# Blackgaurd/pathtracer-cpp

Hardware: AMD Instinct MI355X
Metric: Mray/s (all bounces) + achieved HBM GB/s, Cornell 1024² 10k spp depth-5 (higher is better)
Workload: dtype f32

## Files before the change

### include/pt_hip_debug.h

```cpp
#ifndef PT_HIP_DEBUG_H
#define PT_HIP_DEBUG_H

#include "pt_hip.h"

#ifdef __cplusplus
extern "C" {
#endif

int pt_debug_math(int device, int which, const float* in, int n, float* out);
int pt_debug_sweep(int device, int which, uint32_t lo_bits, uint32_t hi_bits, uint64_t* mismatches,
                   uint32_t* first_bad);
int pt_debug_rgb8(int device, const float* linear_rgb, int32_t res_x, int32_t res_y, float gamma, uint8_t* rgb8);
int pt_debug_rccl_failover(int32_t n_devices, int32_t fail_step, int64_t* out);
int pt_debug_wide_verify(const pt_scene* scene, int32_t width);
int pt_debug_pack_hash(const pt_scene* scene, uint64_t* hash);
int pt_rtc_check(const pt_scene* scene, char* src_out, size_t cap);
int pt_debug_rtc_start(const pt_scene* scene);
int64_t pt_debug_rtc_cache(int32_t op);

int pt_debug_ctx_flags(const pt_ctx* ctx, int32_t out[5]);
int pt_debug_ctx_plan(const pt_ctx* ctx, int64_t out[24]);
int pt_debug_walk_placement(int32_t num_nodes, int32_t num_tris, int32_t tree_depth, int32_t tri_f4,
                            int32_t rec_rows, uint64_t lds_usable, int32_t out[4]);
int pt_debug_scene_dark(const pt_scene* scene);
int pt_debug_emit_reject(const float* box6, const float* org, const float* dir, int64_t n, uint8_t* out);
int pt_debug_emit_slab_reject(const float* box6, const float* org, const float* inv, int64_t n, uint8_t* out);
int pt_debug_emit_box(const pt_scene* scene, float out[6]);
int pt_debug_ctx_emit_reject(const pt_ctx* ctx, int32_t* on, float box[6], uint64_t* early);
int pt_debug_ray_stack(int32_t which, int32_t count, int32_t n, int32_t reserve, int32_t flag);
int64_t pt_debug_counter(int32_t which);

#ifdef __cplusplus
}
#endif
#endif
```

### pathtracer-cpp_amd/csrc/pt_kernel.hip

```cpp
#include <hip/hip_runtime.h>

#include <stdint.h>
#include <stdio.h>
#include <stdlib.h>
#include <string.h>

#include <algorithm>
#include <chrono>
#include <future>
#include <map>
#include <memory>
#include <mutex>
#include <string>
#include <thread>
#include <vector>

#include <atomic>

#include "pt_grad.h"
#include "pt_hip_debug.h"
#include "pt_launch.h"
#include "pt_moments.h"
#include "pt_rtc.h"
#include "pt_trace.h"
// ... 297 lines not shown
    float4* d_nrm = nullptr;
    float4* d_umats = nullptr;
    int32_t* d_rank_tri = nullptr;
    std::vector<f4> flat_host;
    FlatLeaves flat_tab;
    int flat_boxes_padded = 0;
    PackedScene meta;
    bool have_scene = false;
    bool has_specular = false;
    bool albedo_x2 = false;
    bool dark = false;
    EmitBox emit;
    uint64_t last_early = 0;
    void* flat_fast = nullptr;
    int flat_boxes = 0;
    bool rtc_requested = false;
    float* d_radiance = nullptr;
    size_t radiance_floats = 0;
    uint32_t* d_flags = nullptr;
    size_t flags_words = 0;
    float* d_accum = nullptr;
    size_t accum_floats = 0;
    float* d_out = nullptr;
    size_t out_floats = 0;
    unsigned long long* d_ctr = nullptr;
    unsigned long long* d_stamps = nullptr;
    int* d_xstack = nullptr;
    size_t xstack_ints = 0;
    uint8_t* d_rgb8 = nullptr;
    size_t rgb8_bytes = 0;
// ... 228 lines not shown
int batch_at(const RenderPlan& P, int s0) {
    const int left = P.spp - s0;
    if (P.tail <= 0 || left <= P.tail) return std::min(P.batch, left);
    return left <= P.batch + P.tail ? left - P.tail : P.batch;
}

size_t flat_lds_bytes(const pt_ctx* c, const RenderPlan& P, int queue) {
    return sizeof(float4) * (size_t)(3 + 2) * c->meta.num_tris + sizeof(uint16_t) * (size_t)queue * (kBlock / kWave) +
           (sizeof(uint16_t) + sizeof(float)) * (size_t)kBlock * P.rec + sizeof(unsigned long long) * kBlock +
           (sizeof(float4) + sizeof(uint32_t)) * kBlock + P.box_tab_bytes;
}

void plan_flat(const pt_ctx* c, RenderPlan& P) {
    P.pairs = !hook_off("PT_PAIRS");
    P.box_tab_bytes = (sizeof(uint16_t) * (size_t)c->flat_boxes + 3) & ~(size_t)3;
    int queue = P.pairs ? 512 : 0;
    const char* pq = hook_env("PT_PAIR_QUEUE");
    if (P.pairs && pq && *pq) {
        queue = std::max(1, std::min(queue, atoi(pq)));
    } else if (P.pairs && c->lds_usable > 0) {
        auto blocks = [&](int q) { return std::min(8, lds_blocks(c->lds_usable, flat_lds_bytes(c, P, q))); };
        const int want = blocks(kPairQueueMin);
        while (queue > kPairQueueMin && blocks(queue) < want) queue -= 32;
    }
    P.pair_queue = (queue + 3) & ~3;
    P.lds_scene = true;
    P.lds_bytes = flat_lds_bytes(c, P, P.pair_queue);
}

size_t wide_lds_bytes(const pt_ctx* c, const RenderPlan& P, int top) {
// ... 310 lines not shown
            fprintf(stderr,
                    "[stamps] wide timeline: span %.3f ms, first exhaustion at %.3f ms, last wave end %.3f ms after it, "
                    "last exhaustion %.3f ms after it | mean wave life %.3f ms, mean end - own exhaustion %.3f ms\n",
                    (hs[18] - t0) * 1e-5, (ex0 - t0) * 1e-5, (hs[18] - ex0) * 1e-5, (hs[22] - ex0) * 1e-5,
                    hs[20] / w * 1e-5, hs[21] / w * 1e-5);
        }
        const double tot = (double)(hs[0] + hs[5] + hs[3] + hs[4]);
        if (!wide) fprintf(stderr,
                "[stamps] waves %llu  cycles/wave %.3g  start %.1f%%  intersect %.1f%% (box mask %.1f%%, "
                "pair phase %.1f%%)  shade %.1f%%  fold %.1f%%\n",
                hs[6], tot / (double)(hs[6] ? hs[6] : 1), 100 * hs[0] / tot, 100 * hs[5] / tot,
                100 * hs[1] / tot, 100 * hs[2] / tot, 100 * hs[3] / tot, 100 * hs[4] / tot);
        const double it = (double)(hs[7] ? hs[7] : 1);
        if (!wide)
            fprintf(stderr, "[stamps] per flat wave-iteration: pairs %.1f, pair rounds %.2f, max pairs of a lane %.2f, "
                    "rays credited %.2f (%llu wave-iterations)\n",
                hs[8] / it, hs[9] / it, hs[10] / it, (double)h_ctr[1] / it, hs[7]);
        if (!wide)
            fprintf(stderr, "[stamps] camera-ray generator: %.4f runs per wave-iteration, %.2f lanes per run (%llu runs)\n",
                    hs[11] / it, (double)hs[12] / (double)(hs[11] ? hs[11] : 1), hs[11]);
    }
}
#endif

int kernel_path_of(const pt_ctx* c, const RenderPlan& P) {
    return P.use_rtc                ? PT_PATH_FLAT_RTC
           : P.flat && c->flat_fast ? PT_PATH_FLAT_TABLE_FAST
           : P.flat                 ? PT_PATH_FLAT_TABLE
           : P.wide                 ? PT_PATH_WIDE
           : P.lds_scene            ? PT_PATH_TREE_LDS
                                    : PT_PATH_TREE_GLOBAL;
}
// ... 364 lines not shown
    ps.nrm.clear();
    ps.umats.clear();
    ps.nodes.clear();
    ps.tris.clear();
    ps.mats.clear();
    ps.rank_tri.clear();
    c->has_specular = specular;
    c->dark = dark;
    c->emit = emit;
    c->albedo_x2 = false;
    c->flat_fast = nullptr;
    if (flat_eligible(ps) && !hook_off("PT_FLAT_FAST") && leaves_single(ps.leaves, ps.num_leaves) && ps.coords_small &&
        c->dark && albedo_x2)
        c->flat_fast = flat_fast_kernel(specular, ps.num_leaves <= 32);
    c->flat_boxes = 0;
    c->rtc_requested = false;
    c->flat_host = ps.leaves;
    ps.leaves.clear();
    c->meta = ps;
    build_flat_table(c);
    c->rtc_flat = nullptr;
    c->rtc_job = RtcFuture();
    c->rtc_src.clear();
    c->rtc_status = "not a flat scene";
    if (want_rtc) {
        c->rtc_src = std::move(src);
        c->albedo_x2 = albedo_x2;
        c->rtc_requested = true;
        c->flat_boxes = flat_box_pairs(c->flat_host, ps.num_leaves);
        c->rtc_job = job;
        c->rtc_status = "compiling";
        const char* w = hook_env("PT_RTC_WAIT");
        if ((w && *w == '1') || !rtc_async_ready()) rtc_resolve(c, true);
    }
    c->have_scene = true;
    return PT_OK;
}

int pt_rtc_wait(void) { return rtc_wait_all(); }

int pt_ctx_prepare(pt_ctx* c) {
    if (!c) return set_error(PT_E_ARG, "context is NULL");
    if (int rc = ctx_ready(c)) return rc;
    if (c->rtc_job.valid()) {
// ... 1051 lines not shown
    return PT_OK;
}

int pt_debug_ray_stack(int32_t which, int32_t count, int32_t n, int32_t reserve, int32_t flag) {
    switch (which) {
        case 0: return ray_stack_generate(count, n, reserve, flag != 0) ? 1 : 0;
        case 1: return ray_stack_filled(count, n);
        case 2: return ray_stack_dry(count, n) ? 1 : 0;
        case 3: return ray_stack_slot(count, n);
        case 4: return ray_stack_taken(count, n);
        case 5: return ray_stack_done(flag != 0, count, n != 0) ? 1 : 0;
    }
    return set_error(PT_E_ARG, "pt_debug_ray_stack: which = %d", which);
}

int pt_debug_ctx_plan(const pt_ctx* c, int64_t out[24]) {
    if (!c || !out) return set_error(PT_E_ARG, "pt_debug_ctx_plan: NULL argument");
    memcpy(out, c->last_plan, sizeof(c->last_plan));
    return PT_OK;
}

int pt_debug_scene_dark(const pt_scene* scene) {
    PackedScene ps;
    const int rc = pack_scene(scene, ps);
    if (rc) return rc;
    return scene_dark(ps) ? 1 : 0;
}

int pt_debug_math(int device, int which, const float* in, int n, float* out) {
    if (!in || !out || n <= 0 || which < 0 || which > 2) return set_error(PT_E_ARG, "pt_debug_math: bad argument");
// ... 53 lines not shown
```

### pathtracer-cpp_amd/csrc/pt_rtc.h

```cpp
#pragma once

#include <hip/hip_runtime_api.h>

#include <future>
#include <memory>
#include <string>
#include <vector>

#include "pt_internal.h"

namespace pt {

struct RtcCode {
    std::vector<char> code;
    std::string status;
    std::string disk_key;
};
typedef std::shared_future<std::shared_ptr<const RtcCode>> RtcFuture;

int flat_box_pairs(const std::vector<f4>& leaves, int n, std::vector<uint16_t>* tab = nullptr);
bool leaves_single(const std::vector<f4>& leaves, int n);
std::string rtc_flat_source(const std::vector<f4>& leaves, int n, bool specular, bool tri_fast, bool albedo_x2,
                            bool dark, const EmitBox& emit);
RtcFuture rtc_job(const std::string& src);
bool rtc_async_ready();
int rtc_wait_all();
hipFunction_t rtc_load(int device, const std::string& src, const RtcCode& code, std::string& status);

}
```

### pathtracer-cpp_amd/csrc/pt_rtc.hip

```cpp
#include <hip/hip_runtime.h>
#include <hip/hiprtc.h>

#include <dlfcn.h>
#include <errno.h>
#include <fcntl.h>
#include <link.h>
#include <signal.h>
#include <spawn.h>
#include <stdint.h>
#include <stdio.h>
#include <stdlib.h>
#include <string.h>
#include <sys/socket.h>
#include <sys/stat.h>
#include <sys/wait.h>
#include <unistd.h>

#include <algorithm>
#include <atomic>
#include <chrono>
#include <fstream>
#include <future>
#include <limits>
#include <map>
// ... 4 lines not shown
#include <string>
#include <thread>
#include <vector>

extern char** environ;

#include "pt_hip_debug.h"
#include "pt_launch.h"
#include "pt_rtc.h"
#include "pt_sha256.h"
#include "pt_trace.h"

extern "C" const char* pt_rtc_src_trace;
extern "C" const char* pt_rtc_src_math;
extern "C" const char* pt_rtc_src_stack;
extern "C" const char* pt_rtc_src_hip;

namespace pt {

namespace {

std::string hexf(float v) {
    char b[64];
    snprintf(b, sizeof(b), "%af", (double)v);
    return b;
}

std::string litf(float v) {
    if (v == std::numeric_limits<float>::infinity()) return "__builtin_inff()";
    if (v == -std::numeric_limits<float>::infinity()) return "-__builtin_inff()";
    return hexf(v);
}

}

int flat_box_pairs(const std::vector<f4>& leaves, int n, std::vector<uint16_t>* tab) {
    const char* e = hook_env("PT_BOX_PAIRS");
    if (!e || *e != '1') return 0;
    std::map<std::vector<uint32_t>, int> box_id;
    std::vector<std::vector<int>> box_leaves;
    for (int k = 0; k < n; k++) {
        const f4 a = leaves[2 * k], b = leaves[2 * k + 1];
        if (__builtin_bit_cast(int, b.z) != k || __builtin_bit_cast(int, b.w) != k) return 0;
        const std::vector<uint32_t> key = {f2u(a.x), f2u(a.y), f2u(a.z), f2u(a.w), f2u(b.x), f2u(b.y)};
        auto it = box_id.find(key);
        if (it == box_id.end()) {
            it = box_id.emplace(key, (int)box_leaves.size()).first;
            box_leaves.emplace_back();
        }
        box_leaves[it->second].push_back(k);
    }
    for (const auto& l : box_leaves)
        if (l.size() > 2 || l.back() > 254) return 0;
    if (tab) {
        tab->clear();
        for (const auto& l : box_leaves) tab->push_back((uint16_t)(l[0] | ((l.size() > 1 ? l[1] : 0xff) << 8)));
    }
    return (int)box_leaves.size();
}

bool leaves_single(const std::vector<f4>& leaves, int n) {
    for (int k = 0; k < n; k++)
        if (__builtin_bit_cast(int, leaves[2 * k + 1].z) != k || __builtin_bit_cast(int, leaves[2 * k + 1].w) != k)
            return false;
    return true;
}

namespace {

std::string flat_mask_source(const std::vector<f4>& leaves, int n, bool specular, bool tri_fast, bool albedo_x2,
                             bool dark, const EmitBox& emit) {
    std::vector<std::map<uint32_t, int>> planes(3);
    auto plane = [&](int ax, float c) {
// ... 112 lines not shown
            acc += bit;
    }
    acc += "#if PT_MULTI_LEAF_OR\n";
    for (size_t i = 0; i < box_bits.size(); i++) {
        const unsigned long long m = box_bits[i];
        if (__builtin_popcountll(m) < 2) continue;
        const std::string bal = "__builtin_amdgcn_ballot_w64(b" + std::to_string(i) + ")";
        if ((uint32_t)m)
            acc += "        lo = or_if_bit(lo, " + std::to_string((uint32_t)m) + "u, " + bal + ");\n";
        if ((uint32_t)(m >> 32))
            acc += "        hi = or_if_bit(hi, " + std::to_string((uint32_t)(m >> 32)) + "u, " + bal + ");\n";
    }
    acc += "#endif\n";
    acc += "#endif\n";
    std::vector<uint16_t> box_tab;
    const int nbox = flat_box_pairs(leaves, n, &box_tab);
    if (nbox > 0) {
        std::string chain = "        lo = 0;\n        hi = 0;\n";
        for (int u = nbox - 1; u >= 0; u--) {
            const char* w = u >= 32 ? "hi" : "lo";
            chain += std::string("        ") + w + " = shl1_add_bit(" + w + ", __builtin_amdgcn_ballot_w64(b" +
                     std::to_string(u) + "));\n";
        }
        acc = "#if KBOX\n        uint32_t lo, hi;\n" + chain + "#else\n" + acc + "#endif\n";
    }
    acc += "        const unsigned long long m = ((unsigned long long)hi << 32) | lo;\n";
    const bool single = leaves_single(leaves, n);
    const bool sign = tri_fast;
    std::string tabs = "{";
    for (size_t u = 0; u < box_tab.size(); u++) tabs += (u ? ", " : "") + std::to_string(box_tab[u]) + "u";
    tabs += box_tab.empty() ? "0u}" : "}";
    std::string rej = "    using EmitRej = NoEmitReject;\n";
    if (emit.on)
        rej = "    struct EmitRej {\n        static constexpr bool kCompiled = true;\n"
              "        __device__ __forceinline__ static bool on() { return true; }\n"
              "        __device__ __forceinline__ static bool rejected(v3 o, v3 d) {\n"
              "            return emit_reject(v3{" + litf(emit.lo[0]) + ", " + litf(emit.lo[1]) + ", " + litf(emit.lo[2]) +
              "}, v3{" + litf(emit.hi[0]) + ", " + litf(emit.hi[1]) + ", " + litf(emit.hi[2]) + "}, o, d);\n"
              "        }\n"
              "        static constexpr bool kSlab = !PT_EMIT_SIGN_ONLY;\n"
              "        __device__ __forceinline__ static bool rejected_slab(v3 o, v3, v3 inv) {\n"
              "            return emit_slab_reject(v3{" + litf(emit.lo[0]) + ", " + litf(emit.lo[1]) + ", " + litf(emit.lo[2]) +
              "}, v3{" + litf(emit.hi[0]) + ", " + litf(emit.hi[1]) + ", " + litf(emit.hi[2]) + "}, o, inv);\n"
              "        }\n    };\n";
    return std::string("#ifndef PT_FLAT_SIGN_MASK\n#define PT_FLAT_SIGN_MASK 0\n#endif\n#define KSIGN (PT_FLAT_SIGN_MASK && ") +
           (sign ? "1" : "0") + ")\n" + "#define KBOX " + (nbox > 0 ? "(!KSIGN)" : "0") + "\n" +
           "namespace pt {\nstruct SceneBoxMask {\n    static constexpr bool kSignMask = KSIGN;\n"
           "    static constexpr bool kBoxPairs = KBOX;\n    static constexpr bool kCamInvGen = PT_CAM_INV == 2;\n"
           "    static constexpr bool kRayStack = PT_RAY_STACK != 0;\n"
           "    static constexpr int kBoxes = " + std::to_string(nbox) +
           ";\n    static constexpr uint16_t kBoxTab[" + std::to_string(std::max<size_t>(1, box_tab.size())) + "] = " + tabs +
           ";\n    static constexpr bool kMask32 = " +
           (n <= 32 ? "true" : "false") + ";\n    static constexpr bool kSingleTri = " + (single ? "true" : "false") +
           ";\n    static constexpr bool kSpecular = " + (specular ? "true" : "false") +
           ";\n    static constexpr bool kTriFast = " + (tri_fast ? "true" : "false") +
           ";\n    static constexpr bool kAlbedoX2 = " + (albedo_x2 ? "true" : "false") +
           ";\n    static constexpr bool kDarkKnown = true;\n    static constexpr bool kDark = " + (dark ? "true" : "false") +
           ";\n" + rej + "    __device__ __forceinline__ static unsigned long long "
           "mask(const TraceArgs&, v3 o, v3 inv) {\n" +
           body + tests + acc + "        return m;\n    }\n};\n}  // namespace pt\n";
}

struct RtcCache {
    std::mutex mu;
    std::map<std::string, RtcFuture> code;
    std::map<std::pair<int, std::string>, hipFunction_t> funcs;
    std::set<std::string> refused;
// ... 97 lines not shown
        dlclose(h);
    }
    const std::string rtc = lib_of(reinterpret_cast<const void*>(&hiprtcCompileProgram));
    if (!rtc.empty()) libs.push_back(rtc);
    if (runtime) {
        const std::string hip = lib_of(reinterpret_cast<const void*>(&hipModuleLoadData));
        if (!hip.empty()) libs.push_back(hip);
    }
    return libs;
}

std::string rtc_key(const std::string& src) {
    Sha256 k;
    k.update("pathtracer-amd hipRTC code object v1");
    k.update(src.c_str(), src.size() + 1);
    for (const char* h : {pt_rtc_src_trace, pt_rtc_src_math, pt_rtc_src_stack, pt_rtc_src_hip}) k.update(h, strlen(h) + 1);
    for (const std::string& f : rtc_flags()) k.update(f.c_str(), f.size() + 1);
    int maj = 0, mnr = 0;
    (void)hiprtcVersion(&maj, &mnr);
    k.update(std::to_string(maj) + "." + std::to_string(mnr));
    k.update(std::to_string(HIP_VERSION) + " " + HIP_VERSION_GITHASH);
    for (const std::string& lib : rtc_compiler_libs(true)) {
        struct stat st;
        const bool ok = stat(lib.c_str(), &st) == 0;
        k.update(lib + " " + (ok ? std::to_string((long long)st.st_size) + " " + std::to_string((long long)st.st_mtime) : "?"));
    }
    return k.hex();
}

bool rtc_dir_private(const std::string& dir) {
    struct stat st;
// ... 180 lines not shown
    };
    auto get = [fd](void* p, size_t n) {
        char* c = static_cast<char*>(p);
        while (n > 0) {
            const ssize_t r = recv(fd, c, n, 0);
            if (r <= 0) return false;
            c += r;
            n -= (size_t)r;
        }
        return true;
    };
    auto put_str = [&put](const char* str, size_t n) {
        const uint64_t len = n;
        return put(&len, 8) && put(str, n);
    };
    const char* hdrs[] = {pt_rtc_src_trace, pt_rtc_src_math, pt_rtc_src_stack, pt_rtc_src_hip};
    const char* names[] = {"pt_trace.h", "pt_math.h", "pt_raystack.h", "pt_hip.h"};
    const std::vector<std::string> flags = rtc_flags();
    const uint32_t head[3] = {0x51525450u , 4u, (uint32_t)flags.size()};
    bool ok = put(head, 12) && put_str(src.data(), src.size());
    for (int i = 0; ok && i < 4; i++) ok = put_str(names[i], strlen(names[i])) && put_str(hdrs[i], strlen(hdrs[i]));
    for (size_t i = 0; ok && i < flags.size(); i++) ok = put_str(flags[i].data(), flags[i].size());
    uint32_t resp[2] = {0, 0};
    uint64_t n = 0;
    ok = ok && get(resp, 8) && resp[0] == 0x53525450u  && get(&n, 8) && n < ((uint64_t)1 << 30);
    std::vector<char> bytes;
    if (ok) {
        bytes.resize(n);
        ok = n == 0 || get(bytes.data(), n);
    }
    if (!ok) {
        rtc_server_stop(s);
        return false;
    }
    if (resp[1] == 1) {
        out.code = std::move(bytes);
// ... 5 lines not shown

std::shared_ptr<const RtcCode> rtc_compile(const std::string& src, const std::string& key) {
    auto out = std::make_shared<RtcCode>();
    g_rtc_compiles++;
    const auto t0 = std::chrono::steady_clock::now();
    auto done = [&t0]() {
        g_rtc_last_compile_us =
            std::chrono::duration_cast<std::chrono::microseconds>(std::chrono::steady_clock::now() - t0).count();
    };
    if (rtc_server_compile(src, *out)) {
        done();
        g_rtc_server_compiles++;
        if (!out->code.empty()) rtc_disk_store(key, out->code);
        return out;
    }
    const char* hdrs[] = {pt_rtc_src_trace, pt_rtc_src_math, pt_rtc_src_stack, pt_rtc_src_hip};
    const char* names[] = {"pt_trace.h", "pt_math.h", "pt_raystack.h", "pt_hip.h"};
    hiprtcProgram prog;
    if (hiprtcCreateProgram(&prog, src.c_str(), "pt_trace_flat_rtc.hip", 4, hdrs, names) != HIPRTC_SUCCESS) {
        out->status = "hiprtcCreateProgram failed";
        return out;
    }
    const std::vector<std::string> flags = rtc_flags();
    std::vector<const char*> opts;
    for (const std::string& f : flags) opts.push_back(f.c_str());
    if (hiprtcCompileProgram(prog, (int)opts.size(), opts.data()) != HIPRTC_SUCCESS) {
        size_t ls = 0;
        hiprtcGetProgramLogSize(prog, &ls);
        std::string log(ls, '\0');
        if (ls) hiprtcGetProgramLog(prog, &log[0]);
        out->status = "hipRTC compile failed: " + log.substr(0, 400);
    } else {
        size_t cs = 0;
        hiprtcGetCodeSize(prog, &cs);
// ... 149 lines not shown
```

### pathtracer-cpp_amd/csrc/pt_trace.h

```cpp
#pragma once

#include "pt_hip.h"
#include "pt_math.h"
#include "pt_raystack.h"

namespace pt {

constexpr int kBlock = 256;
constexpr int kWave = 64;
static_assert(kRaySlots == kWave, "one prefetched camera ray per lane (pt_raystack.h)");
constexpr int kMaxSpecularIters = 1 << 16;
#ifndef PT_CHUNK
#define PT_CHUNK 1024
#endif
constexpr int kChunk = PT_CHUNK;
static_assert(kChunk >= kWave, "a work-pool refill must cover one claim of every lane of a wave");
constexpr int kMaxFlatLeaves = 64;

#ifndef PT_WAVES
#define PT_WAVES 7
#endif

#ifdef PT_STAMPS
#define PT_STAMP(v)                                  \
// ... 278 lines not shown
        cb = __float_as_int(q.w);
    }
    t_out = t;
    return hit;
}

struct TableBoxMask {
    static constexpr bool kMask32 = false;
    static constexpr bool kSingleTri = false;
    static constexpr bool kSpecular = true;
    static constexpr bool kTriFast = false;
    static constexpr bool kSignMask = false;
    static constexpr bool kAlbedoX2 = false;
    static constexpr bool kDarkKnown = false;
    static constexpr bool kBoxPairs = false;
    static constexpr bool kCamInvGen = false;
    static constexpr bool kRayStack = true;
    static constexpr int kBoxes = 0;
    static constexpr uint16_t kBoxTab[1] = {0};
    static constexpr bool kDark = false;
    using EmitRej = KernargEmitSlabReject;
    __device__ __forceinline__ static unsigned long long mask(const TraceArgs& A, v3 o, v3 inv) {
        const float(*box)[6] = A.flat.box;
        unsigned long long m = 0;
        const int n = A.num_boxes_padded;
        for (int k = 0; k < n; k += 4) {
#pragma unroll
            for (int j = 0; j < 4; j++) {
                const float* b = box[k + j];
                if (slab_hit_finite(v3{b[0], b[1], b[2]}, v3{b[3], b[4], b[5]}, o, inv)) m |= A.flat.bits[k + j];
// ... 32 lines not shown
        const float4 b = lleaves[2 * k + 1];
        const int last = __float_as_int(b.w);
        for (int i = __float_as_int(b.z); i <= last; i++) {
            const float4 t0 = tris[3 * i], t1 = tris[3 * i + 1], t2 = tris[3 * i + 2];
            float tt;
            if (tri_hit(v3{t0.x, t0.y, t0.z}, v3{t0.w, t1.x, t1.y}, v3{t1.z, t1.w, t2.x}, o, d, tt) && tt < t) {
                t = tt;
                hit = i;
            }
        }
    }
    t_out = t;
    return hit;
}

__device__ __forceinline__ int flat_box_loop(unsigned long long mask, const uint16_t* __restrict__ boxtab,
                                             const float4* __restrict__ tris, v3 o, v3 d, float& t_out) {
    int hit = -1;
    float t = 1e30f;
    while (mask) {
        const int u = __builtin_ctzll(mask);
        mask &= mask - 1;
        const uint32_t code = boxtab[u];
        for (int j = 0; j < 2; j++) {
            const uint32_t r = j ? code >> 8 : code & 0xffu;
            if (r == 0xffu) continue;
            const int i = (int)r;
            const float4 t0 = tris[3 * i], t1 = tris[3 * i + 1], t2 = tris[3 * i + 2];
            float tt;
            if (tri_hit(v3{t0.x, t0.y, t0.z}, v3{t0.w, t1.x, t1.y}, v3{t1.z, t1.w, t2.x}, o, d, tt) &&
                (tt < t || (tt == t && i < hit))) {
                t = tt;
                hit = i;
            }
        }
    }
    t_out = t;
    return hit;
}

template <typename BoxMask, typename TriPtr, typename LeafPtr>
__device__ __forceinline__ int intersect_flat(const TraceArgs& A, LeafPtr lleaves, TriPtr tris, v3 o, v3 d, v3 inv,
                                              float& t_out, const uint16_t* __restrict__ boxtab) {
    if constexpr (BoxMask::kBoxPairs) return flat_box_loop(BoxMask::mask(A, o, inv), boxtab, tris, o, d, t_out);
    return flat_tri_loop(BoxMask::mask(A, o, inv), lleaves, tris, o, d, t_out);
}

__device__ __forceinline__ uint32_t wave_incl_scan(uint32_t x) {
    x += (uint32_t)__builtin_amdgcn_update_dpp(0, (int)x, 0x111, 0xf, 0xf, false);
    x += (uint32_t)__builtin_amdgcn_update_dpp(0, (int)x, 0x112, 0xf, 0xf, false);
    x += (uint32_t)__builtin_amdgcn_update_dpp(0, (int)x, 0x114, 0xf, 0xf, false);
    x += (uint32_t)__builtin_amdgcn_update_dpp(0, (int)x, 0x118, 0xf, 0xf, false);
    x += (uint32_t)__builtin_amdgcn_update_dpp(0, (int)x, 0x142, 0xa, 0xf, false);
    x += (uint32_t)__builtin_amdgcn_update_dpp(0, (int)x, 0x143, 0xc, 0xf, false);
    return x;
}

__device__ __forceinline__ void wave_lds_sync() {
    __builtin_amdgcn_fence(__ATOMIC_RELEASE, "wavefront");
    __builtin_amdgcn_wave_barrier();
    __builtin_amdgcn_fence(__ATOMIC_ACQUIRE, "wavefront");
}

__device__ __forceinline__ float lane_float(int addr, float v) {
    return __int_as_float(__builtin_amdgcn_ds_bpermute(addr, __float_as_int(v)));
}

template <typename BoxMask, typename TriPtr, typename LeafPtr>
__device__ __forceinline__ int intersect_flat_pairs(const TraceArgs& A, unsigned long long mask, LeafPtr lleaves,
                                                    TriPtr tris, uint16_t* __restrict__ queue,
                                                    unsigned long long* __restrict__ best, int tid, int lane, v3 o,
                                                    v3 d, float& t_out, const uint16_t* __restrict__ boxtab) {
    const uint32_t c = (uint32_t)__popcll(mask);
    const uint32_t incl = wave_incl_scan(c);
    const uint32_t total = (uint32_t)__builtin_amdgcn_readlane((int)incl, 63);
    if (total > (uint32_t)A.pair_queue) {
        if constexpr (BoxMask::kBoxPairs) return flat_box_loop(mask, boxtab, tris, o, d, t_out);
        return flat_tri_loop(mask, lleaves, tris, o, d, t_out);
    }
    best[tid] = ~0ull;
    uint16_t* at = queue + (incl - c);
    uint32_t tag = (uint32_t)lane << 6;
    asm volatile("" : "+v"(tag));
    if constexpr (BoxMask::kMask32) {
        uint32_t m = (uint32_t)mask;
        while (m) {
            const uint32_t b0 = (uint32_t)__builtin_ctz(m);
            m &= m - 1;
            at[0] = (uint16_t)(tag | b0);
            if (m) {
                at[1] = (uint16_t)(tag | (uint32_t)__builtin_ctz(m));
                m &= m - 1;
            }
            at += 2;
        }
    } else {
        while (mask) {
            const uint32_t b0 = (uint32_t)__builtin_ctzll(mask);
            mask &= mask - 1;
// ... 1225 lines not shown
__device__ __forceinline__ void trace_body_flat(const TraceArgs& A) {
    extern __shared__ float4 lds4[];
    const int tid = threadIdx.x;
    const int lane = tid & (kWave - 1);
    float4* s_tris = lds4;
    float4* s_mats = s_tris + A.num_tri4;
    uint16_t* queues = reinterpret_cast<uint16_t*>(s_mats + A.num_mat4);
    uint16_t* rec_tri = queues + (kBlock / kWave) * A.pair_queue;
    float* rec_cos = reinterpret_cast<float*>(rec_tri + A.rec_size * kBlock);
    unsigned long long* best = reinterpret_cast<unsigned long long*>(rec_cos + A.rec_size * kBlock);
    float4* next_ray = reinterpret_cast<float4*>(best + kBlock);
    uint32_t* next_at = reinterpret_cast<uint32_t*>(next_ray + kBlock);
    uint16_t* boxtab = reinterpret_cast<uint16_t*>(next_at + kBlock);
    if constexpr (BoxMask::kBoxPairs)
        for (int i = tid; i < BoxMask::kBoxes; i += kBlock) boxtab[i] = BoxMask::kBoxTab[i];
    for (int i = tid; i < A.num_tri4; i += kBlock) s_tris[i] = A.tris[i];
    for (int i = tid; i < A.num_mat4; i += kBlock) {
        float4 m = A.mats[i];
        if (BoxMask::kAlbedoX2 && !(i & 1)) m = make_float4(m.x, 2.0f * m.y, 2.0f * m.z, 2.0f * m.w);
        s_mats[i] = m;
    }
    __syncthreads();
    const float4* __restrict__ mats = s_mats;
    const float4* __restrict__ tris = s_tris;
    uint16_t* wq = queues + __builtin_amdgcn_readfirstlane(tid >> 6) * A.pair_queue;
    int* xstk = A.exact_stack + (size_t)blockIdx.x * A.exact_rows * kBlock;

    bool alive = true;
    bool active = false;
    bool has_next = false;
// ... 121 lines not shown
            unsigned long long mask = BoxMask::mask(A, o, inv);
#ifdef PT_EXP_DUP_MASK
            {
                v3 o2 = o;
                asm volatile("" : "+v"(o2.x));
                const unsigned long long m2 = BoxMask::mask(A, o2, inv);
                asm volatile("" ::"v"((uint32_t)m2), "v"((uint32_t)(m2 >> 32)));
            }
#endif
            if (PT_PRIO_MASK) __builtin_amdgcn_s_setprio(0);
            if (!tr) mask = 0ull;
            PT_STAMP(st_b2)
            PT_STAMP_ADD(1, st_b, st_b2)
#ifdef PT_STAMPS
            {
                const uint32_t pc = (uint32_t)__popcll(mask);
                const uint32_t tot = (uint32_t)__builtin_amdgcn_readlane((int)wave_incl_scan(pc), 63);
                int mx = (int)pc;
                for (int off = 32; off > 0; off >>= 1) mx = max(mx, __shfl_xor(mx, off));
                stamp_acc[7] += 1;
                stamp_acc[8] += tot;
                stamp_acc[9] += (tot + 63) / 64;
                stamp_acc[10] += (uint32_t)mx;
            }
#endif
#ifdef PT_EXP_NO_PAIRS
            hit = mask ? __builtin_ctzll(mask) : -1;
            t = 1.0f;
#else
            if (PT_PRIO_PAIRS) __builtin_amdgcn_s_setprio(PT_PRIO_PAIRS);
            hit = intersect_flat_pairs<BoxMask>(A, mask, A.leaves, tris, wq, best, fresh_tid(), lane, o, d, t, boxtab);
            if (PT_PRIO_PAIRS) __builtin_amdgcn_s_setprio(0);
#endif
            PT_STAMP(st_b3)
            PT_STAMP_ADD(2, st_b2, st_b3)
        } else if (tr) {
            if (fast) hit = intersect_flat<BoxMask>(A, A.leaves, tris, o, d, inv, t, boxtab);
            else hit = intersect_tree<false>(A.nodes, tris, xstk, tid, o, d, inv, t);
// ... 391 lines not shown
```

### pathtracer-cpp_amd/ptamd/_lib.py

```python
from __future__ import annotations

import atexit
import ctypes as C
import os
import subprocess
from typing import Optional

PKG_ROOT = os.path.dirname(os.path.dirname(os.path.abspath(__file__)))
REPO_ROOT = os.path.dirname(PKG_ROOT)
LIB_PATH = os.environ.get("PT_LIB") or os.path.join(PKG_ROOT, "lib", "libpt_hip.so")

PT_OK, PT_E_ARG, PT_E_EMPTY, PT_E_HIP, PT_E_IO, PT_E_RUNAWAY = 0, -1, -2, -3, -4, -5
PT_SEED = 1
PT_MAX_DEPTH = 64

EXPORTED = (
    "pt_abi_version", "pt_last_error", "pt_device_count", "pt_bvh_build", "pt_camera_init",
    "pt_ctx_create", "pt_ctx_destroy", "pt_ctx_set_scene", "pt_ctx_prepare", "pt_rtc_wait", "pt_ctx_render", "pt_part_rows",
    "pt_render_f32", "pt_image_to_rgb8", "pt_write_png", "pt_debug_math", "pt_debug_sweep", "pt_scene_validate", "pt_rtc_check",
    "pt_ctx_render_progressive", "pt_ctx_render_rgb8", "pt_rgb8_thresholds", "pt_debug_rgb8",
    "pt_obj_load", "pt_obj_num_tris", "pt_obj_triangles", "pt_obj_warnings", "pt_obj_free",
    "pt_render_f32_devices", "pt_render_rgb8_devices", "pt_scene_info", "pt_debug_wide_verify",
    "pt_debug_rccl_failover", "pt_debug_rtc_cache", "pt_devices_release", "pt_debug_ctx_flags", "pt_debug_counter",
    "pt_debug_scene_dark", "pt_debug_rtc_start", "pt_debug_pack_hash",
    "pt_bvh_intersect", "pt_ctx_intersect", "pt_ctx_render_aov",
    "pt_bvh_trace", "pt_ctx_trace", "pt_debug_ctx_plan", "pt_debug_walk_placement",
    "pt_bvh_trace_grad", "pt_ctx_trace_grad",
    "pt_debug_emit_reject", "pt_debug_emit_box", "pt_debug_ctx_emit_reject", "pt_debug_emit_slab_reject", "pt_debug_ray_stack",
    "pt_ctx_render_moments", "pt_moments_unconverged", "pt_ctx_unconverged", "pt_ctx_render_converge",
    "pt_ctx_render_adaptive",
    "pt_moments_variance", "pt_ctx_moments_variance", "pt_image_denoise", "pt_ctx_denoise", "pt_ctx_render_denoised",
    "pt_image_temporal", "pt_ctx_temporal", "pt_ctx_render_temporal",
    "pt_scene_lights", "pt_bvh_trace_nee", "pt_ctx_trace_nee", "pt_ctx_render_nee",
)
PT_MAX_DEVICES = 16


class pt_bvh_node(C.Structure):
    _fields_ = [("lb", C.c_float * 3), ("rt", C.c_float * 3), ("left", C.c_int32), ("right", C.c_int32),
                ("tri_start", C.c_int32), ("tri_end", C.c_int32)]


class pt_material(C.Structure):
# ... 339 lines not shown
            L.pt_debug_ctx_plan.argtypes = [P, P]
        if hasattr(L, "pt_debug_walk_placement"):
            L.pt_debug_walk_placement.argtypes = [C.c_int32] * 5 + [C.c_uint64, P]
        if hasattr(L, "pt_debug_scene_dark"):
            L.pt_debug_scene_dark.argtypes = [C.POINTER(pt_scene)]
        if hasattr(L, "pt_debug_pack_hash"):
            L.pt_debug_pack_hash.argtypes = [C.POINTER(pt_scene), C.POINTER(C.c_uint64)]
        if hasattr(L, "pt_debug_rtc_start"):
            L.pt_debug_rtc_start.argtypes = [C.POINTER(pt_scene)]
        if hasattr(L, "pt_debug_emit_reject"):
            L.pt_debug_emit_reject.argtypes = [P, P, P, C.c_int64, P]
            L.pt_debug_emit_box.argtypes = [C.POINTER(pt_scene), P]
            L.pt_debug_ctx_emit_reject.argtypes = [P, P, P, P]
        if hasattr(L, "pt_debug_emit_slab_reject"):
            L.pt_debug_emit_slab_reject.argtypes = [P, P, P, C.c_int64, P]
        if hasattr(L, "pt_debug_counter"):
            L.pt_debug_counter.argtypes = [C.c_int32]
            L.pt_debug_counter.restype = C.c_int64
        if L.pt_abi_version() != 3:
            raise RuntimeError("libpt_hip.so ABI version mismatch")
        _lib = L
    return _lib


def check(rc: int) -> int:
    if rc < 0:
        raise PTError(rc, lib().pt_last_error().decode(errors="replace"))
    return rc
```

Measured before the change: 81160.

## Enqueue shared-box triangle pairs from packed box words in flat pair queue

Adds a default-on box-bits mode for the hipRTC flat kernel. The ballot mask is built per bounding box rather than per leaf, so it fits in 32 bits when there are at most 32 boxes. Each box maps to a packed 32-bit LDS word holding one or two triangle ranks plus a retreat offset. The pair enqueue then writes both entries with one branch-light store sequence, two boxes per trip, aiming to cut per-leaf mask bits and enqueue loop trips. The trade-offs are slightly more complex queue writes, a pair count that needs an extra popcount, and reliance on box_put's pointer retreat trick being correct.

Result: no change. 81420, median of 6 (+0.3%).

```diff
diff --git a/include/pt_hip_debug.h b/include/pt_hip_debug.h
--- a/include/pt_hip_debug.h
+++ b/include/pt_hip_debug.h
@@ -28,6 +28,8 @@
 int pt_debug_emit_box(const pt_scene* scene, float out[6]);
 int pt_debug_ctx_emit_reject(const pt_ctx* ctx, int32_t* on, float box[6], uint64_t* early);
 int pt_debug_ray_stack(int32_t which, int32_t count, int32_t n, int32_t reserve, int32_t flag);
+int pt_debug_box_bits(const uint16_t* tab, int32_t nbox, const uint64_t* masks, int64_t n, uint32_t* counts,
+                      uint16_t* queue, int64_t cap, int32_t mutant);
 int64_t pt_debug_counter(int32_t which);
 
 #ifdef __cplusplus
diff --git a/pathtracer-cpp_amd/csrc/pt_boxbits.h b/pathtracer-cpp_amd/csrc/pt_boxbits.h
--- /dev/null
+++ b/pathtracer-cpp_amd/csrc/pt_boxbits.h
@@ -0,0 +1,46 @@
+#pragma once
+
+#if defined(__HIPCC__)
+#define PT_BB_HD __host__ __device__ __forceinline__
+#else
+#define PT_BB_HD inline
+#endif
+
+namespace pt {
+
+constexpr uint32_t kBoxNoSecond = 0x80000000u;
+
+PT_BB_HD uint32_t box_word(uint32_t code) {
+    const uint32_t r0 = code & 0xffu, r1 = (code >> 8) & 0xffu;
+    return r0 | (r1 == 0xffu ? kBoxNoSecond : r1 << 16);
+}
+PT_BB_HD bool box_has_second(uint32_t word) { return (int32_t)word >= 0; }
+PT_BB_HD uint32_t box_rank0(uint32_t word) { return word & 0xffffu; }
+PT_BB_HD uint32_t box_rank1(uint32_t word) { return (word >> 16) & 0x7fffu; }
+PT_BB_HD uint32_t box_pair_count(unsigned long long m, unsigned long long two) {
+    return (uint32_t)__builtin_popcountll(m) + (uint32_t)__builtin_popcountll(m & two);
+}
+PT_BB_HD uint32_t box_tag2(uint32_t lane) { return lane * 0x00400040u; }
+PT_BB_HD uint32_t box_entries(uint32_t word, uint32_t tag2) { return word | tag2; }
+PT_BB_HD int box_retreat_bytes(uint32_t word) { return (int32_t)word >> 30; }
+
+template <bool kSecondAlways = false>
+PT_BB_HD uint16_t* box_put(uint16_t* at, uint32_t word, uint32_t tag2) {
+    const uint32_t e = box_entries(word, tag2);
+    at[0] = (uint16_t)e;
+    if (kSecondAlways || box_has_second(word)) at[1] = (uint16_t)(e >> 16);
+    return reinterpret_cast<uint16_t*>(reinterpret_cast<char*>(at + 2) + box_retreat_bytes(word));
+}
+
+PT_BB_HD constexpr int box_table_words(int boxes) { return boxes + 1; }
+PT_BB_HD int box_lowest(uint32_t m) {
+#if defined(__HIP_DEVICE_COMPILE__)
+    int r;
+    asm("v_ffbl_b32_e32 %0, %1" : "=v"(r) : "v"(m));
+    return r;
+#else
+    return m ? (int)__builtin_ctz(m) : -1;
+#endif
+}
+
+}
diff --git a/pathtracer-cpp_amd/csrc/pt_kernel.hip b/pathtracer-cpp_amd/csrc/pt_kernel.hip
--- a/pathtracer-cpp_amd/csrc/pt_kernel.hip
+++ b/pathtracer-cpp_amd/csrc/pt_kernel.hip
@@ -335,6 +335,7 @@
     uint64_t last_early = 0;
     void* flat_fast = nullptr;
     int flat_boxes = 0;
+    int flat_bit_boxes = 0;
     bool rtc_requested = false;
     float* d_radiance = nullptr;
     size_t radiance_floats = 0;
@@ -593,6 +594,7 @@
 void plan_flat(const pt_ctx* c, RenderPlan& P) {
     P.pairs = !hook_off("PT_PAIRS");
     P.box_tab_bytes = (sizeof(uint16_t) * (size_t)c->flat_boxes + 3) & ~(size_t)3;
+    if (c->flat_bit_boxes > 0) P.box_tab_bytes = sizeof(uint32_t) * (size_t)box_table_words(c->flat_bit_boxes);
     int queue = P.pairs ? 512 : 0;
     const char* pq = hook_env("PT_PAIR_QUEUE");
     if (P.pairs && pq && *pq) {
@@ -933,8 +935,8 @@
         const double it = (double)(hs[7] ? hs[7] : 1);
         if (!wide)
             fprintf(stderr, "[stamps] per flat wave-iteration: pairs %.1f, pair rounds %.2f, max pairs of a lane %.2f, "
-                    "rays credited %.2f (%llu wave-iterations)\n",
-                hs[8] / it, hs[9] / it, hs[10] / it, (double)h_ctr[1] / it, hs[7]);
+                    "enqueue trips %.2f, rays credited %.2f (%llu wave-iterations)\n",
+                hs[8] / it, hs[9] / it, hs[10] / it, hs[13] / it, (double)h_ctr[1] / it, hs[7]);
         if (!wide)
             fprintf(stderr, "[stamps] camera-ray generator: %.4f runs per wave-iteration, %.2f lanes per run (%llu runs)\n",
                     hs[11] / it, (double)hs[12] / (double)(hs[11] ? hs[11] : 1), hs[11]);
@@ -1329,6 +1331,7 @@
         c->dark && albedo_x2)
         c->flat_fast = flat_fast_kernel(specular, ps.num_leaves <= 32);
     c->flat_boxes = 0;
+    c->flat_bit_boxes = 0;
     c->rtc_requested = false;
     c->flat_host = ps.leaves;
     ps.leaves.clear();
@@ -1343,6 +1346,7 @@
         c->albedo_x2 = albedo_x2;
         c->rtc_requested = true;
         c->flat_boxes = flat_box_pairs(c->flat_host, ps.num_leaves);
+        c->flat_bit_boxes = flat_box_bits(c->flat_host, ps.num_leaves);
         c->rtc_job = job;
         c->rtc_status = "compiling";
         const char* w = hook_env("PT_RTC_WAIT");
@@ -2424,6 +2428,37 @@
     return set_error(PT_E_ARG, "pt_debug_ray_stack: which = %d", which);
 }
 
+int pt_debug_box_bits(const uint16_t* tab, int32_t nbox, const uint64_t* masks, int64_t n, uint32_t* counts,
+                      uint16_t* queue, int64_t cap, int32_t mutant) {
+    if (!tab || !masks || !counts || !queue || nbox < 1 || nbox > 64 || n < 0)
+        return set_error(PT_E_ARG, "pt_debug_box_bits: bad argument");
+    unsigned long long two = 0;
+    std::vector<uint32_t> words(nbox);
+    for (int u = 0; u < nbox; u++) {
+        words[u] = box_word(tab[u]);
+        if (box_has_second(words[u])) two |= 1ull << u;
+    }
+    int64_t total = 0;
+    for (int64_t i = 0; i < n; i++) {
+        if (nbox < 64 && (masks[i] >> nbox)) return set_error(PT_E_ARG, "pt_debug_box_bits: mask %lld names no box", (long long)i);
+        counts[i] = box_pair_count(masks[i], two);
+        total += counts[i];
+    }
+    if (cap < total + 1) return set_error(PT_E_ARG, "pt_debug_box_bits: queue of %lld entries, %lld needed", (long long)cap, (long long)total + 1);
+    for (int64_t i = 0; i < cap; i++) queue[i] = 0xffffu;
+    int64_t end = total;
+    for (int64_t i = n - 1; i >= 0; i--) {
+        uint16_t* at = queue + (end - counts[i]);
+        end -= counts[i];
+        const uint32_t tag2 = box_tag2((uint32_t)(i & 63));
+        for (unsigned long long m = masks[i]; m; m &= m - 1) {
+            const uint32_t w = words[__builtin_ctzll(m)];
+            at = mutant ? box_put<true>(at, w, tag2) : box_put<false>(at, w, tag2);
+        }
+    }
+    return PT_OK;
+}
+
 int pt_debug_ctx_plan(const pt_ctx* c, int64_t out[24]) {
     if (!c || !out) return set_error(PT_E_ARG, "pt_debug_ctx_plan: NULL argument");
     memcpy(out, c->last_plan, sizeof(c->last_plan));
diff --git a/pathtracer-cpp_amd/csrc/pt_rtc.h b/pathtracer-cpp_amd/csrc/pt_rtc.h
--- a/pathtracer-cpp_amd/csrc/pt_rtc.h
+++ b/pathtracer-cpp_amd/csrc/pt_rtc.h
@@ -18,7 +18,9 @@
 };
 typedef std::shared_future<std::shared_ptr<const RtcCode>> RtcFuture;
 
+int flat_box_table(const std::vector<f4>& leaves, int n, std::vector<uint16_t>* tab = nullptr);
 int flat_box_pairs(const std::vector<f4>& leaves, int n, std::vector<uint16_t>* tab = nullptr);
+int flat_box_bits(const std::vector<f4>& leaves, int n, std::vector<uint16_t>* tab = nullptr);
 bool leaves_single(const std::vector<f4>& leaves, int n);
 std::string rtc_flat_source(const std::vector<f4>& leaves, int n, bool specular, bool tri_fast, bool albedo_x2,
                             bool dark, const EmitBox& emit);
diff --git a/pathtracer-cpp_amd/csrc/pt_rtc.hip b/pathtracer-cpp_amd/csrc/pt_rtc.hip
--- a/pathtracer-cpp_amd/csrc/pt_rtc.hip
+++ b/pathtracer-cpp_amd/csrc/pt_rtc.hip
@@ -42,6 +42,7 @@
 extern "C" const char* pt_rtc_src_trace;
 extern "C" const char* pt_rtc_src_math;
 extern "C" const char* pt_rtc_src_stack;
+extern "C" const char* pt_rtc_src_boxbits;
 extern "C" const char* pt_rtc_src_hip;
 
 namespace pt {
@@ -62,9 +63,7 @@
 
 }
 
-int flat_box_pairs(const std::vector<f4>& leaves, int n, std::vector<uint16_t>* tab) {
-    const char* e = hook_env("PT_BOX_PAIRS");
-    if (!e || *e != '1') return 0;
+int flat_box_table(const std::vector<f4>& leaves, int n, std::vector<uint16_t>* tab) {
     std::map<std::vector<uint32_t>, int> box_id;
     std::vector<std::vector<int>> box_leaves;
     for (int k = 0; k < n; k++) {
@@ -85,6 +84,18 @@
         for (const auto& l : box_leaves) tab->push_back((uint16_t)(l[0] | ((l.size() > 1 ? l[1] : 0xff) << 8)));
     }
     return (int)box_leaves.size();
+}
+
+int flat_box_pairs(const std::vector<f4>& leaves, int n, std::vector<uint16_t>* tab) {
+    const char* e = hook_env("PT_BOX_PAIRS");
+    if (!e || *e != '1') return 0;
+    return flat_box_table(leaves, n, tab);
+}
+
+int flat_box_bits(const std::vector<f4>& leaves, int n, std::vector<uint16_t>* tab) {
+    const char* e = hook_env("PT_BOX_BITS");
+    if ((e && *e == '0') || flat_box_pairs(leaves, n) > 0) return 0;
+    return flat_box_table(leaves, n, tab);
 }
 
 bool leaves_single(const std::vector<f4>& leaves, int n) {
@@ -227,7 +238,12 @@
     acc += "#endif\n";
     acc += "#endif\n";
     std::vector<uint16_t> box_tab;
-    const int nbox = flat_box_pairs(leaves, n, &box_tab);
+    const int nbox = flat_box_table(leaves, n, &box_tab);
+    const bool box_pairs = flat_box_pairs(leaves, n) > 0;
+    const bool bits_on = flat_box_bits(leaves, n) > 0;
+    unsigned long long two = 0;
+    for (size_t u = 0; u < box_tab.size(); u++)
+        if ((box_tab[u] >> 8) != 0xff) two |= 1ull << u;
     if (nbox > 0) {
         std::string chain = "        lo = 0;\n        hi = 0;\n";
         for (int u = nbox - 1; u >= 0; u--) {
@@ -235,7 +251,7 @@
             chain += std::string("        ") + w + " = shl1_add_bit(" + w + ", __builtin_amdgcn_ballot_w64(b" +
                      std::to_string(u) + "));\n";
         }
-        acc = "#if KBOX\n        uint32_t lo, hi;\n" + chain + "#else\n" + acc + "#endif\n";
+        acc = "#if KBOX || KBITS\n        uint32_t lo, hi;\n" + chain + "#else\n" + acc + "#endif\n";
     }
     acc += "        const unsigned long long m = ((unsigned long long)hi << 32) | lo;\n";
     const bool single = leaves_single(leaves, n);
@@ -257,13 +273,17 @@
               "}, v3{" + litf(emit.hi[0]) + ", " + litf(emit.hi[1]) + ", " + litf(emit.hi[2]) + "}, o, inv);\n"
               "        }\n    };\n";
     return std::string("#ifndef PT_FLAT_SIGN_MASK\n#define PT_FLAT_SIGN_MASK 0\n#endif\n#define KSIGN (PT_FLAT_SIGN_MASK && ") +
-           (sign ? "1" : "0") + ")\n" + "#define KBOX " + (nbox > 0 ? "(!KSIGN)" : "0") + "\n" +
+           (sign ? "1" : "0") + ")\n" + "#define KBOX " + (box_pairs ? "(!KSIGN)" : "0") + "\n" +
+           "#ifndef PT_BOX_BITS\n#define PT_BOX_BITS 1\n#endif\n" +
+           "#define KBITS (PT_BOX_BITS && !KSIGN && !KBOX && " + (bits_on ? "1" : "0") + ")\n" +
            "namespace pt {\nstruct SceneBoxMask {\n    static constexpr bool kSignMask = KSIGN;\n"
-           "    static constexpr bool kBoxPairs = KBOX;\n    static constexpr bool kCamInvGen = PT_CAM_INV == 2;\n"
+           "    static constexpr bool kBoxPairs = KBOX;\n    static constexpr bool kBoxBits = KBITS;\n"
+           "    static constexpr unsigned long long kTwo = " + std::to_string(two) + "ull;\n"
+           "    static constexpr bool kCamInvGen = PT_CAM_INV == 2;\n"
            "    static constexpr bool kRayStack = PT_RAY_STACK != 0;\n"
            "    static constexpr int kBoxes = " + std::to_string(nbox) +
            ";\n    static constexpr uint16_t kBoxTab[" + std::to_string(std::max<size_t>(1, box_tab.size())) + "] = " + tabs +
-           ";\n    static constexpr bool kMask32 = " +
+           ";\n    static constexpr bool kMask32 = " + (nbox > 0 && nbox <= 32 && n > 32 ? "KBITS ? true : " : "") +
            (n <= 32 ? "true" : "false") + ";\n    static constexpr bool kSingleTri = " + (single ? "true" : "false") +
            ";\n    static constexpr bool kSpecular = " + (specular ? "true" : "false") +
            ";\n    static constexpr bool kTriFast = " + (tri_fast ? "true" : "false") +
@@ -391,7 +411,7 @@
     Sha256 k;
     k.update("pathtracer-amd hipRTC code object v1");
     k.update(src.c_str(), src.size() + 1);
-    for (const char* h : {pt_rtc_src_trace, pt_rtc_src_math, pt_rtc_src_stack, pt_rtc_src_hip}) k.update(h, strlen(h) + 1);
+    for (const char* h : {pt_rtc_src_trace, pt_rtc_src_math, pt_rtc_src_stack, pt_rtc_src_boxbits, pt_rtc_src_hip}) k.update(h, strlen(h) + 1);
     for (const std::string& f : rtc_flags()) k.update(f.c_str(), f.size() + 1);
     int maj = 0, mnr = 0;
     (void)hiprtcVersion(&maj, &mnr);
@@ -602,12 +622,12 @@
         const uint64_t len = n;
         return put(&len, 8) && put(str, n);
     };
-    const char* hdrs[] = {pt_rtc_src_trace, pt_rtc_src_math, pt_rtc_src_stack, pt_rtc_src_hip};
-    const char* names[] = {"pt_trace.h", "pt_math.h", "pt_raystack.h", "pt_hip.h"};
+    const char* hdrs[] = {pt_rtc_src_trace, pt_rtc_src_math, pt_rtc_src_stack, pt_rtc_src_boxbits, pt_rtc_src_hip};
+    const char* names[] = {"pt_trace.h", "pt_math.h", "pt_raystack.h", "pt_boxbits.h", "pt_hip.h"};
     const std::vector<std::string> flags = rtc_flags();
-    const uint32_t head[3] = {0x51525450u , 4u, (uint32_t)flags.size()};
+    const uint32_t head[3] = {0x51525450u , 5u, (uint32_t)flags.size()};
     bool ok = put(head, 12) && put_str(src.data(), src.size());
-    for (int i = 0; ok && i < 4; i++) ok = put_str(names[i], strlen(names[i])) && put_str(hdrs[i], strlen(hdrs[i]));
+    for (int i = 0; ok && i < 5; i++) ok = put_str(names[i], strlen(names[i])) && put_str(hdrs[i], strlen(hdrs[i]));
     for (size_t i = 0; ok && i < flags.size(); i++) ok = put_str(flags[i].data(), flags[i].size());
     uint32_t resp[2] = {0, 0};
     uint64_t n = 0;
@@ -643,10 +663,10 @@
         if (!out->code.empty()) rtc_disk_store(key, out->code);
         return out;
     }
-    const char* hdrs[] = {pt_rtc_src_trace, pt_rtc_src_math, pt_rtc_src_stack, pt_rtc_src_hip};
-    const char* names[] = {"pt_trace.h", "pt_math.h", "pt_raystack.h", "pt_hip.h"};
+    const char* hdrs[] = {pt_rtc_src_trace, pt_rtc_src_math, pt_rtc_src_stack, pt_rtc_src_boxbits, pt_rtc_src_hip};
+    const char* names[] = {"pt_trace.h", "pt_math.h", "pt_raystack.h", "pt_boxbits.h", "pt_hip.h"};
     hiprtcProgram prog;
-    if (hiprtcCreateProgram(&prog, src.c_str(), "pt_trace_flat_rtc.hip", 4, hdrs, names) != HIPRTC_SUCCESS) {
+    if (hiprtcCreateProgram(&prog, src.c_str(), "pt_trace_flat_rtc.hip", 5, hdrs, names) != HIPRTC_SUCCESS) {
         out->status = "hiprtcCreateProgram failed";
         return out;
     }
diff --git a/pathtracer-cpp_amd/csrc/pt_trace.h b/pathtracer-cpp_amd/csrc/pt_trace.h
--- a/pathtracer-cpp_amd/csrc/pt_trace.h
+++ b/pathtracer-cpp_amd/csrc/pt_trace.h
@@ -3,6 +3,7 @@
 #include "pt_hip.h"
 #include "pt_math.h"
 #include "pt_raystack.h"
+#include "pt_boxbits.h"
 
 namespace pt {
 
@@ -316,6 +317,8 @@
     static constexpr bool kAlbedoX2 = false;
     static constexpr bool kDarkKnown = false;
     static constexpr bool kBoxPairs = false;
+    static constexpr bool kBoxBits = false;
+    static constexpr unsigned long long kTwo = 0;
     static constexpr bool kCamInvGen = false;
     static constexpr bool kRayStack = true;
     static constexpr int kBoxes = 0;
@@ -378,6 +381,7 @@
     return hit;
 }
 
+template <bool kWords = false>
 __device__ __forceinline__ int flat_box_loop(unsigned long long mask, const uint16_t* __restrict__ boxtab,
                                              const float4* __restrict__ tris, v3 o, v3 d, float& t_out) {
     int hit = -1;
@@ -385,7 +389,13 @@
     while (mask) {
         const int u = __builtin_ctzll(mask);
         mask &= mask - 1;
-        const uint32_t code = boxtab[u];
+        uint32_t code;
+        if constexpr (kWords) {
+            const uint32_t w = reinterpret_cast<const uint32_t*>(boxtab)[u + 1];
+            code = box_rank0(w) | (box_has_second(w) ? box_rank1(w) : 0xffu) << 8;
+        } else {
+            code = boxtab[u];
+        }
         for (int j = 0; j < 2; j++) {
             const uint32_t r = j ? code >> 8 : code & 0xffu;
             if (r == 0xffu) continue;
@@ -407,6 +417,7 @@
 __device__ __forceinline__ int intersect_flat(const TraceArgs& A, LeafPtr lleaves, TriPtr tris, v3 o, v3 d, v3 inv,
                                               float& t_out, const uint16_t* __restrict__ boxtab) {
     if constexpr (BoxMask::kBoxPairs) return flat_box_loop(BoxMask::mask(A, o, inv), boxtab, tris, o, d, t_out);
+    if constexpr (BoxMask::kBoxBits) return flat_box_loop<true>(BoxMask::mask(A, o, inv), boxtab, tris, o, d, t_out);
     return flat_tri_loop(BoxMask::mask(A, o, inv), lleaves, tris, o, d, t_out);
 }
 
@@ -430,23 +441,53 @@
     return __int_as_float(__builtin_amdgcn_ds_bpermute(addr, __float_as_int(v)));
 }
 
+#ifndef PT_BOX_TRIP
+#define PT_BOX_TRIP 2
+#endif
 template <typename BoxMask, typename TriPtr, typename LeafPtr>
 __device__ __forceinline__ int intersect_flat_pairs(const TraceArgs& A, unsigned long long mask, LeafPtr lleaves,
                                                     TriPtr tris, uint16_t* __restrict__ queue,
                                                     unsigned long long* __restrict__ best, int tid, int lane, v3 o,
                                                     v3 d, float& t_out, const uint16_t* __restrict__ boxtab) {
-    const uint32_t c = (uint32_t)__popcll(mask);
+    const uint32_t c = BoxMask::kBoxBits ? box_pair_count(mask, BoxMask::kTwo) : (uint32_t)__popcll(mask);
     const uint32_t incl = wave_incl_scan(c);
     const uint32_t total = (uint32_t)__builtin_amdgcn_readlane((int)incl, 63);
     if (total > (uint32_t)A.pair_queue) {
         if constexpr (BoxMask::kBoxPairs) return flat_box_loop(mask, boxtab, tris, o, d, t_out);
+        if constexpr (BoxMask::kBoxBits) return flat_box_loop<true>(mask, boxtab, tris, o, d, t_out);
         return flat_tri_loop(mask, lleaves, tris, o, d, t_out);
     }
     best[tid] = ~0ull;
     uint16_t* at = queue + (incl - c);
     uint32_t tag = (uint32_t)lane << 6;
-    asm volatile("" : "+v"(tag));
-    if constexpr (BoxMask::kMask32) {
+    if constexpr (!BoxMask::kBoxBits) asm volatile("" : "+v"(tag));
+    if constexpr (BoxMask::kBoxBits) {
+        const uint32_t* __restrict__ words = reinterpret_cast<const uint32_t*>(boxtab) + 1;
+        uint32_t tag2 = box_tag2((uint32_t)lane);
+        asm volatile("" : "+v"(tag2));
+        if constexpr (BoxMask::kMask32) {
+            uint32_t m = (uint32_t)mask;
+            while (m) {
+                const uint32_t w0 = words[__builtin_ctz(m)];
+                m &= m - 1;
+                if constexpr (PT_BOX_TRIP == 2) {
+                    const bool more = m != 0;
+                    const uint32_t w1 = words[box_lowest(m)];
+                    m &= m - 1;
+                    at = box_put(at, w0, tag2);
+                    if (more) at = box_put(at, w1, tag2);
+                } else {
+                    at = box_put(at, w0, tag2);
+                }
+            }
+        } else {
+            while (mask) {
+                const uint32_t w0 = words[__builtin_ctzll(mask)];
+                mask &= mask - 1;
+                at = box_put(at, w0, tag2);
+            }
+        }
+    } else if constexpr (BoxMask::kMask32) {
         uint32_t m = (uint32_t)mask;
         while (m) {
             const uint32_t b0 = (uint32_t)__builtin_ctz(m);
@@ -1702,6 +1743,9 @@
     uint16_t* boxtab = reinterpret_cast<uint16_t*>(next_at + kBlock);
     if constexpr (BoxMask::kBoxPairs)
         for (int i = tid; i < BoxMask::kBoxes; i += kBlock) boxtab[i] = BoxMask::kBoxTab[i];
+    if constexpr (BoxMask::kBoxBits)
+        for (int i = tid; i < box_table_words(BoxMask::kBoxes); i += kBlock)
+            reinterpret_cast<uint32_t*>(boxtab)[i] = i > 0 ? box_word(BoxMask::kBoxTab[i - 1]) : kBoxNoSecond;
     for (int i = tid; i < A.num_tri4; i += kBlock) s_tris[i] = A.tris[i];
     for (int i = tid; i < A.num_mat4; i += kBlock) {
         float4 m = A.mats[i];
@@ -1853,7 +1897,7 @@
             PT_STAMP_ADD(1, st_b, st_b2)
 #ifdef PT_STAMPS
             {
-                const uint32_t pc = (uint32_t)__popcll(mask);
+                const uint32_t pc = BoxMask::kBoxBits ? box_pair_count(mask, BoxMask::kTwo) : (uint32_t)__popcll(mask);
                 const uint32_t tot = (uint32_t)__builtin_amdgcn_readlane((int)wave_incl_scan(pc), 63);
                 int mx = (int)pc;
                 for (int off = 32; off > 0; off >>= 1) mx = max(mx, __shfl_xor(mx, off));
@@ -1861,6 +1905,11 @@
                 stamp_acc[8] += tot;
                 stamp_acc[9] += (tot + 63) / 64;
                 stamp_acc[10] += (uint32_t)mx;
+                int trips = ((int)pc + 1) / 2;
+                if constexpr (BoxMask::kBoxBits)
+                    trips = BoxMask::kMask32 ? (__popcll(mask) + PT_BOX_TRIP - 1) / PT_BOX_TRIP : __popcll(mask);
+                for (int off = 32; off > 0; off >>= 1) trips = max(trips, __shfl_xor(trips, off));
+                stamp_acc[13] += (uint32_t)trips;
             }
 #endif
 #ifdef PT_EXP_NO_PAIRS
diff --git a/pathtracer-cpp_amd/ptamd/_lib.py b/pathtracer-cpp_amd/ptamd/_lib.py
--- a/pathtracer-cpp_amd/ptamd/_lib.py
+++ b/pathtracer-cpp_amd/ptamd/_lib.py
@@ -27,6 +27,7 @@
     "pt_bvh_trace", "pt_ctx_trace", "pt_debug_ctx_plan", "pt_debug_walk_placement",
     "pt_bvh_trace_grad", "pt_ctx_trace_grad",
     "pt_debug_emit_reject", "pt_debug_emit_box", "pt_debug_ctx_emit_reject", "pt_debug_emit_slab_reject", "pt_debug_ray_stack",
+    "pt_debug_box_bits",
     "pt_ctx_render_moments", "pt_moments_unconverged", "pt_ctx_unconverged", "pt_ctx_render_converge",
     "pt_ctx_render_adaptive",
     "pt_moments_variance", "pt_ctx_moments_variance", "pt_image_denoise", "pt_ctx_denoise", "pt_ctx_render_denoised",
@@ -396,6 +397,8 @@
             L.pt_debug_ctx_emit_reject.argtypes = [P, P, P, P]
         if hasattr(L, "pt_debug_emit_slab_reject"):
             L.pt_debug_emit_slab_reject.argtypes = [P, P, P, C.c_int64, P]
+        if hasattr(L, "pt_debug_box_bits"):
+            L.pt_debug_box_bits.argtypes = [P, C.c_int32, P, C.c_int64, P, P, C.c_int64, C.c_int32]
         if hasattr(L, "pt_debug_counter"):
             L.pt_debug_counter.argtypes = [C.c_int32]
             L.pt_debug_counter.restype = C.c_int64
```
